# youmi-zym/GO-SLAM

Measured on NVIDIA H100. Metric: keyframe-BA-updates/s, higher is better.
Workload: dtype f16 corr (f32 accumulate) / f32 BA (f64 solve)

## Files before the change

go-slam_b200/csrc/ba.cu:

```cuda
#include "common.cuh"
#include <cstring>
#include "se3.cuh"
#include <algorithm>
#include <cstdio>
#include <mutex>
#include <cooperative_groups.h>

namespace {

constexpr int kTP = 128;
constexpr int kNRed = 27;
constexpr float kAlpha = 0.05f;

struct BaWs {
  int* slot_of_frame;
  int* kx;
  int* counts;
  int* row_ptr;
  int* edge_idx;
  int* entry_ptr;
  int* entry_code;
  int* pair_ptr;
  int* edge_j;
  float* Eij;
  float* Ei;
  float* Q;
  float* w;
  float* part;
  double* sys;
  double* chol;
  double* rhs;
  float* dx;
  int ntiles;
};

struct BaDims {
  int N, num, ht, wd, hw, t0, t1, P, n;
};

size_t ba_layout(const BaDims& d, void* base, size_t cap, BaWs* ws) {
  GsArena a(base, cap);
  const int ntiles = gs_cdiv(d.hw, kTP);
  BaWs w{};
  w.slot_of_frame = a.take<int>(d.num);
  w.kx = a.take<int>(d.num);
  w.counts = a.take<int>(8);
  w.row_ptr = a.take<int>(d.num + 1);
  w.edge_idx = a.take<int>(d.N > 0 ? d.N : 1);
  w.entry_ptr = a.take<int>(d.num + 1);
  w.entry_code = a.take<int>(d.num + d.N);
  w.pair_ptr = a.take<int>(d.num + 1);
  w.edge_j = a.take<int>(d.N > 0 ? d.N : 1);
  w.Eij = a.take<float>((size_t)(d.N > 0 ? d.N : 1) * 6 * d.hw);
  w.Ei = a.take<float>((size_t)d.num * 6 * d.hw);
  w.Q = a.take<float>((size_t)d.num * d.hw);
  w.w = a.take<float>((size_t)d.num * d.hw);
  w.part = a.take<float>((size_t)(d.N > 0 ? d.N : 1) * ntiles * (kTP / 32) * kNRed);
  w.sys = a.take<double>((size_t)d.n * d.n + d.n);
  w.chol = a.take<double>((size_t)d.n * d.n);
  w.rhs = a.take<double>(d.n > 0 ? d.n : 1);
  w.dx = a.take<float>((size_t)(d.P > 0 ? d.P : 1) * 6);
  w.ntiles = ntiles;
  if (ws) *ws = w;
  return a.off;
}

constexpr int kPrepThreads = 1024;
constexpr int kPrepMaxFrames = 4 * kPrepThreads;

__device__ int prep_excl_scan(int* a, int n, int* wsum ) {
  const int tid = threadIdx.x, lane = tid & 31, warp = tid >> 5;
  const int per = (n + (int)blockDim.x - 1) / (int)blockDim.x;
  const int base = tid * per;
  int loc[4], s = 0;
#pragma unroll
  for (int q = 0; q < 4; ++q) {
    loc[q] = s;
    if (q < per && base + q < n) s += a[base + q];
  }
  int inc = s;
#pragma unroll
  for (int o = 1; o < 32; o <<= 1) {
    const int t = __shfl_up_sync(0xffffffffu, inc, o);
    if (lane >= o) inc += t;
  }
  if (lane == 31) wsum[warp] = inc;
  __syncthreads();
  if (warp == 0) {
    const int w = lane < ((int)blockDim.x >> 5) ? wsum[lane] : 0;
    int winc = w;
#pragma unroll
    for (int o = 1; o < 32; o <<= 1) {
      const int t = __shfl_up_sync(0xffffffffu, winc, o);
      if (lane >= o) winc += t;
    }
    wsum[lane] = winc - w;
    if (lane == 31) wsum[32] = winc;
  }
  __syncthreads();
  const int off = wsum[warp] + inc - s;
#pragma unroll
  for (int q = 0; q < 4; ++q)
    if (q < per && base + q < n) a[base + q] = off + loc[q];
  const int total = wsum[32];
  __syncthreads();
  return total;
}

__global__ void __launch_bounds__(kPrepThreads)
ba_prep_kernel(const int64_t* __restrict__ ii, const int64_t* __restrict__ jj, BaDims d, BaWs ws, int zero,
               int eta_rows) {
  extern __shared__ int sm[];
  const int tid = threadIdx.x, nt = blockDim.x;
  if (zero) {
    const size_t nsys = (size_t)d.n * d.n + d.n;
    for (size_t i = tid; i < nsys; i += nt) ws.sys[i] = 0.0;
    if (tid == 0) ws.counts[3] = 0;
  }
  int* a = sm;
  int* b = sm + d.num;
  int* c = b + d.num + 1;
  int* wsum = c + d.num;
  for (int f = tid; f < d.num; f += nt) { a[f] = (f >= d.t0 && f < d.t1) ? 1 : 0; b[f] = 0; }
  __syncthreads();
  for (int e = tid; e < d.N; e += nt) {
    const int f = (int)ii[e];
    if (f >= 0 && f < d.num) { a[f] = 1; atomicAdd(&b[f], 1); }
    ws.edge_j[e] = (int)jj[e];
  }
  __syncthreads();
  for (int f = tid; f < d.num; f += nt) c[f] = a[f];
  __syncthreads();
  const int M = prep_excl_scan(c, d.num, wsum);
  for (int f = tid; f < d.num; f += nt) {
    if (a[f]) { ws.slot_of_frame[f] = c[f]; ws.kx[c[f]] = f; }
    else ws.slot_of_frame[f] = -1;
  }
  if (tid == 0) {
    ws.counts[0] = M;
    ws.counts[4] = (eta_rows == 0 || eta_rows == 1 || eta_rows == M || eta_rows == -d.num) ? 0 : 1;
  }
  const int n_listed = prep_excl_scan(b, d.num, wsum);
  if (tid == 0) b[d.num] = n_listed;
  __syncthreads();
  for (int f = tid; f <= d.num; f += nt) ws.row_ptr[f] = b[f];
  for (int e = tid; e < d.N; e += nt) {
    const int f = (int)ii[e];
    if (f < 0 || f >= d.num) continue;
    int rank = 0;
    for (int q = 0; q < e; ++q) rank += ((int)ii[q] == f);
    ws.edge_idx[b[f] + rank] = e;
  }
  __syncthreads();
  for (int k = tid; k < d.num; k += nt) {
    int ne = 0;
    if (k < M) {
      const int f = ws.kx[k];
      ne = (f >= d.t0 && f < d.t1) ? 1 : 0;
      for (int r = b[f]; r < b[f + 1]; ++r) {
        const int j = (int)jj[ws.edge_idx[r]];
        ne += (j >= d.t0 && j < d.t1) ? 1 : 0;
      }
    }
    a[k] = ne;
    c[k] = ne * (ne + 1) / 2;
  }
  __syncthreads();
  const int n_entries = prep_excl_scan(a, d.num, wsum);
  const int n_pairs = prep_excl_scan(c, d.num, wsum);
  for (int k = tid; k < M; k += nt) {
    const int f = ws.kx[k];
    int eo = a[k];
    ws.entry_ptr[k] = eo;
    ws.pair_ptr[k] = c[k];
    if (f >= d.t0 && f < d.t1) ws.entry_code[eo++] = -(f - d.t0 + 1);
    for (int r = b[f]; r < b[f + 1]; ++r) {
      const int e = ws.edge_idx[r];
      const int j = (int)jj[e];
      if (j >= d.t0 && j < d.t1) ws.entry_code[eo++] = e;
    }
  }
  if (tid == 0) {
    ws.entry_ptr[M] = n_entries;
    ws.pair_ptr[M] = n_pairs;
    ws.counts[1] = n_entries;
    ws.counts[2] = n_pairs;
  }
}

__device__ __forceinline__ float warp_transpose_reduce32(float (&v)[32], int lane) {
#pragma unroll
  for (int half = 16; half >= 1; half >>= 1) {
    const bool up = (lane & half) != 0;
#pragma unroll
    for (int i = 0; i < half; ++i) {
      const float send = up ? v[i] : v[i + half];
      const float keep = up ? v[i + half] : v[i];
      v[i] = keep + __shfl_xor_sync(0xffffffffu, send, half);
    }
  }
  return v[0];
}

struct BaIn {
  const float* poses; const float* disps; const float* intr; const float* disps_sens;
  const float* targets; const float* weights; const float* eta; int eta_rows;
  const int64_t* ii; const int64_t* jj;
};

__device__ __forceinline__ void linearize_tile(const BaIn& in, const BaDims& d, const BaWs& ws,
                                               int motion_only, int k, int wt) {
  const float* poses = in.poses; const float* disps = in.disps;
  const float* __restrict__ intr = in.intr; const float* __restrict__ disps_sens = in.disps_sens;
  const float* __restrict__ targets = in.targets; const float* __restrict__ weights = in.weights;
  const float* __restrict__ eta = in.eta; const int eta_rows = in.eta_rows;
  const int f = ws.kx[k];
  const int lane = threadIdx.x & 31;
  const int px = wt * 32 + lane;
  const bool act = px < d.hw;

  const float fx = intr[0], fy = intr[1], cx = intr[2], cy = intr[3];
  const float u = (float)(px % d.wd), v = (float)(px / d.wd);
  const float di = act ? disps[(size_t)f * d.hw + px] : 1.0f;
  float Xi[4] = {(u - cx) / fx, (v - cy) / fy, 1.0f, di};

  float C = 0.f, wz = 0.f;
  float Ei[6] = {0.f, 0.f, 0.f, 0.f, 0.f, 0.f};

  const int r0 = ws.row_ptr[f], r1 = ws.row_ptr[f + 1];
  float pi[7];
#pragma unroll
  for (int c = 0; c < 7; ++c) pi[c] = poses[7 * (size_t)f + c];
  int e1 = 0, j1 = f, e2 = 0, j2 = f;
  if (r0 < r1) { e1 = ws.edge_idx[r0]; j1 = ws.edge_j[e1]; }
  if (r0 + 1 < r1) { e2 = ws.edge_idx[r0 + 1]; j2 = ws.edge_j[e2]; }
  float nx[4] = {0.f, 0.f, 0.f, 0.f}, pn[7] = {0.f, 0.f, 0.f, 0.f, 0.f, 0.f, 1.f};
  if (r0 < r1) {
    if (act) {
      const size_t o = ((size_t)e1 * 2) * d.hw + px;
      nx[0] = targets[o]; nx[1] = targets[o + d.hw]; nx[2] = weights[o]; nx[3] = weights[o + d.hw];
    }
#pragma unroll
    for (int c = 0; c < 7; ++c) pn[c] = poses[7 * (size_t)j1 + c];
  }
  for (int r = r0; r < r1; ++r) {
    const int e = e1, jx = j1;
    const float tu = nx[0], tv = nx[1], qu = nx[2], qv = nx[3];
    float pj[7];
#pragma unroll
    for (int c = 0; c < 7; ++c) pj[c] = pn[c];
    e1 = e2; j1 = j2;
    if (r + 1 < r1) {
      if (act) {
        const size_t o = ((size_t)e1 * 2) * d.hw + px;
        nx[0] = targets[o]; nx[1] = targets[o + d.hw]; nx[2] = weights[o]; nx[3] = weights[o + d.hw];
      }
#pragma unroll
      for (int c = 0; c < 7; ++c) pn[c] = poses[7 * (size_t)j1 + c];
    }
    if (r + 2 < r1) { e2 = ws.edge_idx[r + 2]; j2 = ws.edge_j[e2]; }
    const bool stereo = (jx == f);
    GsSE3 G;
    if (stereo) {
      G.t[0] = -0.1f; G.t[1] = 0.f; G.t[2] = 0.f;
      G.q[0] = 0.f; G.q[1] = 0.f; G.q[2] = 0.f; G.q[3] = 1.f;
    } else {
      gs_rel(pi, pi + 3, pj, pj + 3, G);
    }

    float Xj[4];
    gs_act4(G, Xi, Xj);
    const float x = Xj[0], y = Xj[1], h = Xj[3];
    const bool behind = Xj[2] < GS_MIN_DEPTH;
    const float dd = behind ? 0.0f : __frcp_rn(Xj[2]);
    const float d2 = dd * dd;
    float wu = (behind || !act) ? 0.0f : (float)(.001 * (double)qu);
    float wv = (behind || !act) ? 0.0f : (float)(.001 * (double)qv);
    const float ru = tu - (fx * dd * x + cx);
    const float rv = tv - (fy * dd * y + cy);

    float Ju[6], Jv[6];
    Ju[0] = fx * (h * dd);       Ju[1] = fx * 0.f;
    Ju[2] = fx * (-x * h * d2);  Ju[3] = fx * (-x * y * d2);
    Ju[4] = fx * (1 + x * x * d2);  Ju[5] = fx * (-y * dd);
    Jv[0] = fy * 0.f;            Jv[1] = fy * (h * dd);
    Jv[2] = fy * (-y * h * d2);  Jv[3] = fy * (-1 - y * y * d2);
    Jv[4] = fy * (x * y * d2);   Jv[5] = fy * (x * dd);
    const float Jzu = fx * (G.t[0] * dd - G.t[2] * (x * d2));
    const float Jzv = fy * (G.t[1] * dd - G.t[2] * (y * d2));

    C += wu * Jzu * Jzu;  C += wv * Jzv * Jzv;
    wz += wu * ru * Jzu;  wz += wv * rv * Jzv;
    if (stereo) { wu = 0.f; wv = 0.f; }

    float val[32];
    {
      int l = 0;
#pragma unroll
      for (int a = 0; a < 6; ++a)
#pragma unroll
        for (int b = a; b < 6; ++b) val[l++] = wu * Ju[a] * Ju[b] + wv * Jv[a] * Jv[b];
#pragma unroll
      for (int a = 0; a < 6; ++a) val[21 + a] = wu * ru * Ju[a] + wv * rv * Jv[a];
#pragma unroll
      for (int a = kNRed; a < 32; ++a) val[a] = 0.f;
    }
    const float tot = warp_transpose_reduce32(val, lane);
    if (lane < kNRed)
      ws.part[((size_t)e * ws.ntiles * (kTP / 32) + wt) * kNRed + lane] = tot;

    if (!motion_only) {
      float Ee[6], Eii[6];
#pragma unroll
      for (int a = 0; a < 6; ++a) Ee[a] = wu * Jzu * Ju[a] + wv * Jzv * Jv[a];
      gs_adjT(G, Ee, Eii);
      if (act) {
#pragma unroll
        for (int a = 0; a < 6; ++a) {
          ws.Eij[((size_t)e * 6 + a) * d.hw + px] = Ee[a];
          Ei[a] -= Eii[a];
        }
      }
    }
  }

  if (!motion_only && act) {
    const float ds = disps_sens[(size_t)f * d.hw + px];
    const float m = (ds > 0.f) ? 1.0f : 0.0f;
    const int er = (eta_rows == 1) ? 0 : (eta_rows < 0 ? f : k);
    const float et = eta[(size_t)er * d.hw + px];
    C = C + m * kAlpha + (1.0f - m) * et;
    wz = wz - m * kAlpha * (di - ds);
    const size_t o = (size_t)k * d.hw + px;
    ws.Q[o] = 1.0f / C;
    ws.w[o] = wz;
#pragma unroll
    for (int a = 0; a < 6; ++a) ws.Ei[((size_t)k * 6 + a) * d.hw + px] = Ei[a];
  }
}

__global__ void __launch_bounds__(kTP)
ba_linearize_kernel(BaIn in, BaDims d, BaWs ws, int motion_only) {
  if ((int)blockIdx.y >= ws.counts[0] || ws.counts[4]) return;
  linearize_tile(in, d, ws, motion_only, blockIdx.y, blockIdx.x * (kTP / 32) + (threadIdx.x >> 5));
}

struct SysSmem {
  float red[8][64];
  double redd[8][32];
  double Hs[36], Ms[36], Ts[36], vs[6];
};

template <int NT>
__device__ __forceinline__ void system_items(const float* poses, const int64_t* __restrict__ ii,
                                             const int64_t* __restrict__ jj, const BaDims& d,
                                             const BaWs& ws, int motion_only, int bid, int nb,
                                             SysSmem& sm) {
  float (*red)[64] = sm.red;
  double* Hs = sm.Hs; double* Ms = sm.Ms; double* Ts = sm.Ts; double* vs = sm.vs;
  const int tid = threadIdx.x, lane = tid & 31, warp = tid >> 5;
  const int M = ws.counts[0];
  const int npairs = motion_only ? 0 : ws.counts[2];
  constexpr int kChunk = 4 * NT;
  const int nchunk = (d.hw + kChunk - 1) / kChunk;
  double* H = ws.sys;
  double* bvec = ws.sys + (size_t)d.n * d.n;

  for (int e = nb - 1 - bid; e < d.N; e += nb) {
    const int ix = (int)ii[e], jx = (int)jj[e];
    const int pi = ix - d.t0, pj = jx - d.t0;
    const bool vi_ok = pi >= 0 && pi < d.P, vj_ok = pj >= 0 && pj < d.P;
    if ((!vi_ok && !vj_ok) || ix < 0 || ix >= d.num) continue;
    {
      double ps = 0.0;
      if (lane < kNRed) {
        const int nparts = ws.ntiles * (kTP / 32);
        const float* pp = ws.part + (size_t)e * nparts * kNRed + lane;
#pragma unroll 8
        for (int t = warp; t < nparts; t += NT / 32) ps += (double)pp[(size_t)t * kNRed];
      }
      sm.redd[warp][lane] = ps;
    }
    __syncthreads();
    if (tid < kNRed) {
      double s = 0.0;
#pragma unroll
      for (int wq = 0; wq < NT / 32; ++wq) s += sm.redd[wq][tid];
      if (tid < 21) {
        int a = 0, l = tid;
        while (l >= 6 - a) { l -= 6 - a; ++a; }
        const int b = a + l;
        Hs[a * 6 + b] = s; Hs[b * 6 + a] = s;
      } else {
        vs[tid - 21] = s;
      }
    }
    if (tid >= 32 && tid < 38) {
      const int c = tid - 32;
      GsSE3 G;
      gs_edge_pose(poses, ix, jx, G);
      float X[6] = {0.f, 0.f, 0.f, 0.f, 0.f, 0.f}, Y[6];
      X[c] = 1.0f;
      gs_adjT(G, X, Y);
      for (int r = 0; r < 6; ++r) Ms[r * 6 + c] = (double)Y[r];
    }
    __syncthreads();
    if (tid < 36) {
      const int r = tid / 6, c = tid % 6;
      double s = 0.0;
      for (int q = 0; q < 6; ++q) s += Ms[r * 6 + q] * Hs[q * 6 + c];
      Ts[tid] = s;
    }
    __syncthreads();
    if (tid < 36) {
      const int r = tid / 6, c = tid % 6;
      if (vi_ok) {
        double s = 0.0;
        for (int q = 0; q < 6; ++q) s += Ts[r * 6 + q] * Ms[c * 6 + q];
        atomicAdd(&H[(size_t)(6 * pi + r) * d.n + 6 * pi + c], s);
      }
      if (vi_ok && vj_ok) {
        atomicAdd(&H[(size_t)(6 * pi + r) * d.n + 6 * pj + c], -Ts[r * 6 + c]);
        atomicAdd(&H[(size_t)(6 * pj + r) * d.n + 6 * pi + c], -Ts[c * 6 + r]);
      }
      if (vj_ok) atomicAdd(&H[(size_t)(6 * pj + r) * d.n + 6 * pj + c], Hs[r * 6 + c]);
    } else if (tid >= 64 && tid < 70) {
      const int r = tid - 64;
      if (vj_ok) atomicAdd(&bvec[6 * pj + r], vs[r]);
      if (vi_ok) {
        double s = 0.0;
        for (int q = 0; q < 6; ++q) s += Ms[r * 6 + q] * vs[q];
        atomicAdd(&bvec[6 * pi + r], -s);
      }
    }
    __syncthreads();
  }

  const int total = npairs * nchunk;
  const int per = (total + nb - 1) / nb;
  const int u0 = bid * per;
  const int u1 = min(total, u0 + per);
  int cur = -1, pa = 0, pb = 0;
  bool diag = false;
  const float* Ea = nullptr; const float* Eb = nullptr; const float* Qk = nullptr; const float* wk = nullptr;
  float acc[64];
  auto flush = [&]() {
    float lo32[32], hi32[32];
#pragma unroll
    for (int i = 0; i < 32; ++i) { lo32[i] = acc[i]; hi32[i] = acc[32 + i]; }
    const float s0 = warp_transpose_reduce32(lo32, lane);
    const float s1 = warp_transpose_reduce32(hi32, lane);
    red[warp][lane] = s0;
    red[warp][32 + lane] = s1;
    __syncthreads();
    if (tid < 42) {
      double s = 0.0;
#pragma unroll
      for (int wq = 0; wq < NT / 32; ++wq) s += (double)red[wq][tid];
      if (tid < 36) {
        const int r = tid / 6, c = tid % 6;
        atomicAdd(&H[(size_t)(6 * pa + r) * d.n + 6 * pb + c], -s);
        if (!diag) atomicAdd(&H[(size_t)(6 * pb + c) * d.n + 6 * pa + r], -s);
      } else {
        atomicAdd(&bvec[6 * pa + (tid - 36)], -s);
      }
    }
    __syncthreads();
  };
  for (int u = u0; u < u1; ++u) {
    const int p = u / nchunk;
    const int px0 = (u - p * nchunk) * kChunk;
    const int px1 = min(d.hw, px0 + kChunk);
    if (p != cur) {
      if (cur >= 0) flush();
      cur = p;
      int k;
      if (M <= 32) {
        const int v = lane < M ? ws.pair_ptr[lane] : 0x7fffffff;
        k = __popc(__ballot_sync(0xffffffffu, v <= p)) - 1;
      } else {
        int lo = 0, hi = M;
        while (hi - lo > 1) {
          const int mid = (lo + hi) >> 1;
          if (ws.pair_ptr[mid] <= p) lo = mid; else hi = mid;
        }
        k = lo;
      }
      const int e0 = ws.entry_ptr[k];
      const int ne = ws.entry_ptr[k + 1] - e0;
      int q = p - ws.pair_ptr[k];
      int a = 0;
      while (q >= ne - a) { q -= ne - a; ++a; }
      const int b = a + q;
      const int ca = ws.entry_code[e0 + a];
      const int cb = ws.entry_code[e0 + b];
      Ea = (ca >= 0) ? ws.Eij + (size_t)ca * 6 * d.hw : ws.Ei + (size_t)k * 6 * d.hw;
      Eb = (cb >= 0) ? ws.Eij + (size_t)cb * 6 * d.hw : ws.Ei + (size_t)k * 6 * d.hw;
      pa = (ca >= 0) ? ws.edge_j[ca] - d.t0 : -ca - 1;
      pb = (cb >= 0) ? ws.edge_j[cb] - d.t0 : -cb - 1;
      Qk = ws.Q + (size_t)k * d.hw;
      wk = ws.w + (size_t)k * d.hw;
      diag = a == b;
#pragma unroll
      for (int i = 0; i < 64; ++i) acc[i] = 0.f;
    }
    float qv[kChunk / NT], wv[kChunk / NT], ea[kChunk / NT][6], eb[kChunk / NT][6];
#pragma unroll
    for (int v = 0; v < kChunk / NT; ++v) {
      const int px = px0 + tid + v * NT;
      const bool ok = px < px1;
      qv[v] = ok ? Qk[px] : 0.f;
      wv[v] = (ok && diag) ? wk[px] : 0.f;
#pragma unroll
      for (int r = 0; r < 6; ++r) {
        ea[v][r] = ok ? Ea[(size_t)r * d.hw + px] : 0.f;
        eb[v][r] = ok ? Eb[(size_t)r * d.hw + px] : 0.f;
      }
    }
#pragma unroll
    for (int v = 0; v < kChunk / NT; ++v) {
#pragma unroll
      for (int r = 0; r < 6; ++r) ea[v][r] *= qv[v];
#pragma unroll
      for (int r = 0; r < 6; ++r)
#pragma unroll
        for (int c = 0; c < 6; ++c) acc[r * 6 + c] += ea[v][r] * eb[v][c];
#pragma unroll
      for (int r = 0; r < 6; ++r) acc[36 + r] += ea[v][r] * wv[v];
    }
  }
  if (cur >= 0) flush();
}

__global__ void __launch_bounds__(256)
ba_system_kernel(const float* poses, const int64_t* __restrict__ ii,
                 const int64_t* __restrict__ jj, BaDims d, BaWs ws, int motion_only) {
  __shared__ SysSmem sm;
  if (ws.counts[4]) return;
  system_items<256>(poses, ii, jj, d, ws, motion_only, blockIdx.x, gridDim.x, sm);
}

constexpr int kMaxPeers = 8;
struct SysSrc {
  const double* p[kMaxPeers];
  int n;
  const unsigned* flags;
  unsigned epoch;
  int* timeout;
};
struct PeerRows {
  float* p[kMaxPeers];
  int n;
};

__device__ __forceinline__ double sys_at(const SysSrc& s, size_t i) {
  double x[kMaxPeers];
#pragma unroll
  for (int r = 0; r < kMaxPeers; ++r) x[r] = r < s.n ? __ldcg(s.p[r] + i) : 0.0;
  double v = x[0];
#pragma unroll
  for (int r = 1; r < kMaxPeers; ++r) v += x[r];
  return v;
}

__device__ __forceinline__ void peer_wait(const unsigned* flags, int n, unsigned epoch, int* timeout) {
  if (n > 1 && (int)threadIdx.x < n) {
    const long long t0 = clock64();
    unsigned v;
    do {
      asm volatile("ld.acquire.sys.global.u32 %0, [%1];" : "=r"(v) : "l"(flags + threadIdx.x) : "memory");
      if ((int)(v - epoch) >= 0) break;
      if (clock64() - t0 > (1ll << 32)) { if (timeout) *timeout = 1; break; }
    } while (true);
  }
  __syncthreads();
}

__global__ void ba_peer_wait_kernel(const unsigned* flags, int n, unsigned epoch, int* timeout) {
  peer_wait(flags, n, epoch, timeout);
}

__global__ void ba_peer_signal_kernel(PeerRows flag_rows, int slot, unsigned epoch) {
  __threadfence_system();
  if ((int)threadIdx.x < flag_rows.n) {
    unsigned* dst = reinterpret_cast<unsigned*>(flag_rows.p[threadIdx.x]) + slot;
    asm volatile("st.release.sys.global.u32 [%0], %1;" ::"l"(dst), "r"(epoch) : "memory");
  }
}

__device__ __forceinline__ void solve_finish(float* poses, const BaDims& d, const BaWs& ws,
                                             const double* x, int fail, float* dx_out,
                                             int* status_out, int tid, int nt) {
  for (int i = tid; i < d.n; i += nt) {
    const float val = fail ? 0.0f : (float)x[i];
    ws.dx[i] = val;
    if (dx_out) dx_out[i] = val;
  }
  if (tid == 0 && status_out) *status_out = fail;
}

__device__ __forceinline__ void bad_argument_step(const BaDims& d, const BaWs& ws, float* dx_out,
                                                  int* status_out, int tid, int nt) {
  for (int i = tid; i < d.n; i += nt) {
    ws.dx[i] = 0.f;
    if (dx_out) dx_out[i] = 0.f;
  }
  if (tid == 0 && status_out) *status_out = 2;
}

__device__ __forceinline__ void retract_poses(float* poses, const BaDims& d, const BaWs& ws, int tid,
                                              int nt) {
  for (int k = tid; k < d.P; k += nt) {
    float* p = poses + 7 * (size_t)(d.t0 + k);
    float t1[3], q1[4];
    gs_retr(ws.dx + 6 * k, p, p + 3, t1, q1);
    p[0] = t1[0]; p[1] = t1[1]; p[2] = t1[2];
    p[3] = q1[0]; p[4] = q1[1]; p[5] = q1[2]; p[6] = q1[3];
  }
}

struct SolveSmem {
  double Lblk[16][15];
  double xs[6];
  int failed;
};

#ifdef GOSLAM_BA_PROBE
__device__ long long g_solve_probe[8];
__device__ int g_phase_cycles[2][1024];
#define SOLVE_PROBE(slot) do { if (threadIdx.x == 0) g_solve_probe[slot] = clock64(); } while (0)
#else
#define SOLVE_PROBE(slot) do {} while (0)
#endif

__device__ __forceinline__ void solve_small(float* poses, const BaDims& d, const BaWs& ws,
                                            const SysSrc& sys_in, float lm, float ep, float* dx_out,
                                            int* status_out, double* smd, SolveSmem& ss) {
  double* xs = ss.xs;
  int& failed = ss.failed;
  const int n = d.n, P = d.P, tid = threadIdx.x, lane = tid & 31;
  double* __restrict__ A = smd;
  double* __restrict__ invd = smd + (size_t)(n + 1) * n;
  SOLVE_PROBE(0);
  float pose_old[7] = {0.f, 0.f, 0.f, 0.f, 0.f, 0.f, 1.f};
  if (tid < P) {
#pragma unroll
    for (int c = 0; c < 7; ++c) pose_old[c] = poses[7 * (size_t)(d.t0 + tid) + c];
  }
  {
    const int tot = (n + 1) * n;
    for (int base = 0; base < tot; base += 128 * 16) {
      double v[16];
#pragma unroll
      for (int u = 0; u < 16; ++u) {
        const int idx = base + tid + 128 * u;
        const int r = idx / n, c = idx - r * n;
        v[u] = (idx < tot && (c <= r || r == n)) ? sys_at(sys_in, idx) : 0.0;
      }
#pragma unroll
      for (int u = 0; u < 16; ++u) {
        const int idx = base + tid + 128 * u;
        const int r = idx / n, c = idx - r * n;
        if (idx < tot && (c <= r || r == n)) {
          double val = v[u];
          if (r == c) val += (double)ep + (double)lm * val;
          A[idx] = val;
        }
      }
    }
  }
  if (tid == 0) failed = 0;
  __syncthreads();
  SOLVE_PROBE(1);

  bool bad = false;
  for (int jb = 0; jb < P; ++jb) {
    const int j0 = 6 * jb;
    double l[6][6];
#pragma unroll
    for (int r = 0; r < 6; ++r)
#pragma unroll
      for (int c = 0; c <= r; ++c) l[r][c] = A[(j0 + r) * n + j0 + c];
#pragma unroll
    for (int k = 0; k < 6; ++k) {
      double dkk = l[k][k];
#pragma unroll
      for (int m = 0; m < k; ++m) dkk -= l[k][m] * l[k][m];
      bad = bad || !(dkk > 0.0);
      const double inv = rsqrt(dkk);
      l[k][k] = inv;
#pragma unroll
      for (int r = k + 1; r < 6; ++r) {
// ... 385 lines not shown
          double* out = rowp + c * 36 + a * 6;
#pragma unroll
          for (int b = 0; b < 6; ++b) {
            double v = out[b];
#pragma unroll
            for (int k = 0; k < 6; ++k) v -= li[k] * Lc[b * 6 + k];
            acc[b] = v;
          }
#pragma unroll
          for (int b = 0; b < 6; ++b) out[b] = acc[b];
        }
      }
      for (int it = ut; it < (P - 1 - jb) * 6; it += un) {
        const int c = jb + 1 + it / 6, b = it % 6;
        const double* Lc = panel + (size_t)c * 36 + b * 6;
        double v = rhs[6 * c + b];
#pragma unroll
        for (int k = 0; k < 6; ++k) v -= xs[k] * Lc[k];
        rhs[6 * c + b] = v;
      }
    }
    CL_PROBE(2);
    cluster.sync();
    CL_PROBE(3);
  }

  {
    for (int jb = P - 1; jb >= 0; --jb) {
      const int owner = jb % kCl, lo = jb / kCl;
      if (q == owner) {
        const double* Ld = rows + cl_row_off(q, lo) + jb * 36;
        if (tid == 0) {
          double v6[6], x[6];
#pragma unroll
          for (int k = 0; k < 6; ++k) {
            const double s01 = inbox[0 * 6 + k] + inbox[1 * 6 + k], s23 = inbox[2 * 6 + k] + inbox[3 * 6 + k];
            const double s45 = inbox[4 * 6 + k] + inbox[5 * 6 + k], s67 = inbox[6 * 6 + k] + inbox[7 * 6 + k];
            v6[k] = rhs[6 * jb + k] - ((s01 + s23) + (s45 + s67));
          }
          int nf = 0;
#pragma unroll
          for (int k = 0; k < 6; ++k) {
            double v = Ld[k * 6 + k] * v6[k];
#pragma unroll
            for (int m = k + 1; m < 6; ++m) v += Ld[m * 6 + k] * v6[m];
            x[k] = v;
            nf |= !isfinite(v);
          }
#pragma unroll
          for (int k = 0; k < 6; ++k) { xs[k] = x[k]; ws.dx[6 * jb + k] = (float)x[k]; }
          if (nf) failed = 1;
        }
        __syncthreads();
        const double* rowp = rows + cl_row_off(q, lo);
        const int cpush = jb < kCl ? jb : kCl;
        if (tid < cpush * 6) {
          const int c = jb - 1 - tid / 6, k = tid % 6;
          const double* blk = rowp + c * 36;
          double v = ps[6 * c + k];
#pragma unroll
          for (int m = 0; m < 6; ++m) v += blk[m * 6 + k] * xs[m];
          ps[6 * c + k] = v;
          cluster.map_shared_rank(inbox, c % kCl)[q * 6 + k] = v;
        }
        for (int it = tid; it < (jb - cpush) * 6; it += kClT) {
          const int c = it / 6, k = it % 6;
          const double* blk = rowp + c * 36;
          double v = ps[6 * c + k];
#pragma unroll
          for (int m = 0; m < 6; ++m) v += blk[m * 6 + k] * xs[m];
          ps[6 * c + k] = v;
        }
      }
      CL_PROBE(5);
      cluster.sync();
      CL_PROBE(6);
    }
  }
#ifdef GOSLAM_BA_PROBE
  if (tid == 0 && (q == 0 || q == 5))
    printf("[cluster solve probe cta %d, P=%d] panel+push %lld | barrier1 %lld | update (factor hidden) %lld | barrier2 %lld | "
           "backward work %lld | backward barrier %lld (cycles)\n", q, P, pc[0], pc[1], pc[2], pc[3], pc[5], pc[6]);
#endif
  if (q == 0) {
    __shared__ int any_fail;
    if (tid == 0) {
      int f = 0;
      for (int oq = 0; oq < kCl; ++oq) f |= *cluster.map_shared_rank(&failed, oq);
      any_fail = f;
    }
    __syncthreads();
    const int fail = any_fail;
    for (int i = tid; i < n; i += kClT) {
      const float val = fail ? 0.0f : ws.dx[i];
      ws.dx[i] = val;
      if (dx_out) dx_out[i] = val;
    }
    if (tid == 0 && status_out) *status_out = fail;
    __syncthreads();
    retract_poses(poses, d, ws, tid, kClT);
  }
  cluster.sync();
}

__device__ __forceinline__ void backsub_tile(float* disps, const BaDims& d, const BaWs& ws,
                                             int owner_lo, int owner_hi, float* dz_out, int k,
                                             int wt, const PeerRows* peers = nullptr) {
  const int f = ws.kx[k];
  if (f < owner_lo || f >= owner_hi) return;
  const int px = wt * 32 + (threadIdx.x & 31);
  if (px >= d.hw) return;
  float acc = 0.f;
  {
    const int ix = f - d.t0;
    if (ix > 0 && ix < d.P) {
      float dw = 0.f;
#pragma unroll
      for (int a = 0; a < 6; ++a) dw += ws.Ei[((size_t)k * 6 + a) * d.hw + px] * ws.dx[6 * ix + a];
      acc += dw;
    }
  }
  for (int r = ws.row_ptr[f]; r < ws.row_ptr[f + 1]; ++r) {
    const int e = ws.edge_idx[r];
    const int ix = ws.edge_j[e] - d.t0;
    if (ix <= 0 || ix >= d.P) continue;
    float dw = 0.f;
#pragma unroll
    for (int a = 0; a < 6; ++a) dw += ws.Eij[((size_t)e * 6 + a) * d.hw + px] * ws.dx[6 * ix + a];
    acc += dw;
  }
  const size_t o = (size_t)k * d.hw + px;
  const float dz = ws.Q[o] * (ws.w[o] - acc);
  const float nv = disps[(size_t)f * d.hw + px] + dz;
  disps[(size_t)f * d.hw + px] = nv;
  if (peers)
    for (int r = 0; r < peers->n; ++r)
      if (peers->p[r] != disps) peers->p[r][(size_t)f * d.hw + px] = nv;
  if (dz_out) dz_out[(size_t)f * d.hw + px] = dz;
}

__global__ void __launch_bounds__(kTP)
ba_backsub_kernel(float* disps, BaDims d, BaWs ws, int owner_lo, int owner_hi, float* dz_out, const PeerRows peers) {
  if ((int)blockIdx.y >= ws.counts[0] || ws.counts[4]) return;
  backsub_tile(disps, d, ws, owner_lo, owner_hi, dz_out, blockIdx.y, blockIdx.x * (kTP / 32) + (threadIdx.x >> 5),
               peers.n > 1 ? &peers : nullptr);
}

#ifdef GOSLAM_BA_PROBE
#define BA_PROBE(slot) do { if (threadIdx.x == 0 && blockIdx.x == 0) probe[slot] = clock64(); } while (0)
#else
#define BA_PROBE(slot) do {} while (0)
#endif

__device__ __forceinline__ void grid_barrier(unsigned* counter, unsigned& epoch) {
  __syncthreads();
  ++epoch;
  if (threadIdx.x == 0) {
    __threadfence();
    atomicAdd(counter, 1u);
    const unsigned target = epoch * gridDim.x;
    unsigned v;
    do {
      asm volatile("ld.acquire.gpu.global.u32 %0, [%1];" : "=r"(v) : "l"(counter) : "memory");
    } while (v < target);
    __threadfence();
  }
  __syncthreads();
}

__global__ void __launch_bounds__(kTP)
ba_persistent_kernel(float* poses, float* disps, BaIn in, BaDims d, BaWs ws, int iterations, float lm,
                     float ep, int motion_only, float* dx_out, float* dz_out, int* status_out,
                     unsigned* barrier) {
  extern __shared__ double smd[];
  __shared__ SysSmem sys_sm;
  __shared__ SolveSmem solve_sm;
  unsigned epoch = 0;
#ifdef GOSLAM_BA_PROBE
  __shared__ long long probe[8];
#endif
  const int M = ws.counts[0];
  const int nwt = ws.ntiles * (kTP / 32);
  const int units = M * nwt;
  const int ufirst = (threadIdx.x >> 5) * gridDim.x + blockIdx.x, ustep = (kTP / 32) * gridDim.x;
  const size_t nsys = (size_t)d.n * d.n + d.n;
  if (dz_out) {
    const size_t ndz = (size_t)d.num * d.hw;
    for (size_t i = (size_t)blockIdx.x * kTP + threadIdx.x; i < ndz; i += (size_t)gridDim.x * kTP) dz_out[i] = 0.f;
  }
  if (ws.counts[4]) {
    if (blockIdx.x == 0) {
      bad_argument_step(d, ws, dx_out, nullptr, threadIdx.x, kTP);
      if (status_out) for (int it = threadIdx.x; it < iterations; it += kTP) status_out[it] = 2;
    }
    return;
  }
  for (int it = 0; it < iterations; ++it) {
    BA_PROBE(0);
#ifdef GOSLAM_BA_PROBE
    const long long tl0 = clock64();
#endif
    for (int u = ufirst; u < units; u += ustep) {
      const int k = u / nwt, wt = u - k * nwt;
      if (it > 0 && !motion_only) backsub_tile(disps, d, ws, 0, d.num, dz_out, k, wt);
      linearize_tile(in, d, ws, motion_only, k, wt);
    }
#ifdef GOSLAM_BA_PROBE
    if (threadIdx.x == 0 && blockIdx.x < 1024) g_phase_cycles[0][blockIdx.x] = (int)(clock64() - tl0);
#endif
    BA_PROBE(1);
    grid_barrier(barrier, epoch);
    BA_PROBE(2);
#ifdef GOSLAM_BA_PROBE
    const long long ts0 = clock64();
#endif
    system_items<kTP>(poses, in.ii, in.jj, d, ws, motion_only, blockIdx.x, gridDim.x, sys_sm);
#ifdef GOSLAM_BA_PROBE
    if (threadIdx.x == 0 && blockIdx.x < 1024) g_phase_cycles[1][blockIdx.x] = (int)(clock64() - ts0);
#endif
    BA_PROBE(3);
    grid_barrier(barrier, epoch);
    BA_PROBE(4);
    if (blockIdx.x == 0) {
      SysSrc local{};
      local.p[0] = ws.sys; local.n = 1;
      solve_small(poses, d, ws, local, lm, ep, dx_out, status_out ? status_out + it : nullptr, smd,
                  solve_sm);
      __syncthreads();
      for (size_t i = threadIdx.x; i < nsys; i += kTP) ws.sys[i] = 0.0;
    }
    BA_PROBE(5);
    grid_barrier(barrier, epoch);
    BA_PROBE(6);
#ifdef GOSLAM_BA_PROBE
    if (threadIdx.x == 0 && blockIdx.x == 0 && it == iterations - 1) {
      for (int ph = 0; ph < 2; ++ph) {
        int mx = 0, arg = 0;
        for (int b = 0; b < (int)gridDim.x && b < 1024; ++b)
          if (g_phase_cycles[ph][b] > mx) { mx = g_phase_cycles[ph][b]; arg = b; }
        printf("[phase %d] slowest block %d: %d cycles; blocks 0/100/200/244/250/270/290/295: %d %d %d %d %d %d %d %d\n", ph, arg,
               mx, g_phase_cycles[ph][0], g_phase_cycles[ph][100], g_phase_cycles[ph][200], g_phase_cycles[ph][244],
               g_phase_cycles[ph][250], g_phase_cycles[ph][270], g_phase_cycles[ph][290], g_phase_cycles[ph][295]);
      }
    }
    if (threadIdx.x == 0 && blockIdx.x == 0)
      printf("[solve probe it=%d] load %lld | factor %lld | backward %lld | finish+retract %lld\n", it,
             g_solve_probe[1] - g_solve_probe[0], g_solve_probe[2] - g_solve_probe[1],
             g_solve_probe[3] - g_solve_probe[2], g_solve_probe[4] - g_solve_probe[3]);
    if (threadIdx.x == 0 && blockIdx.x == 0)
      printf("[ba probe it=%d] linearize %lld | barrier %lld | system %lld | barrier %lld | solve %lld | barrier %lld (cycles)\n",
             it, probe[1] - probe[0], probe[2] - probe[1], probe[3] - probe[2], probe[4] - probe[3],
             probe[5] - probe[4], probe[6] - probe[5]);
#endif
  }
  if (!motion_only)
    for (int u = ufirst; u < units; u += ustep) {
      const int k = u / nwt, wt = u - k * nwt;
      backsub_tile(disps, d, ws, 0, d.num, dz_out, k, wt);
    }
}

bool make_dims(int N, int num, int ht, int wd, int t0, int t1, BaDims* d) {
  if (N < 0 || num <= 0 || num > 4096 || ht <= 0 || wd <= 0) return false;
  d->N = N; d->num = num; d->ht = ht; d->wd = wd; d->hw = ht * wd;
  d->t0 = t0; d->t1 = t1; d->P = t1 - t0 > 0 ? t1 - t0 : 0; d->n = 6 * d->P;
  if (t0 < 0 || t1 > num) return false;
  return true;
}

constexpr int kSmemSolveMaxN = 160;
constexpr int kWarpSolveMaxN = 96;
constexpr int kMaxDevices = 64;
constexpr size_t kClusterSmemMax = 226 * 1024;

struct BaDevice {
  bool ready = false;
  int sms = 0;
  int blocks_per_sm = 0;
};

void ba_persistent_kernel_attrs(BaDevice* dv, int dev) {
  int occ = 0, coop = 0;
  const size_t smem_max = ((size_t)kWarpSolveMaxN * kWarpSolveMaxN + 2 * kWarpSolveMaxN) * sizeof(double);
  cudaDeviceGetAttribute(&dv->sms, cudaDevAttrMultiProcessorCount, dev);
  cudaDeviceGetAttribute(&coop, cudaDevAttrCooperativeLaunch, dev);
  cudaFuncSetAttribute(ba_persistent_kernel, cudaFuncAttributeMaxDynamicSharedMemorySize, (int)smem_max);
  cudaOccupancyMaxActiveBlocksPerMultiprocessor(&occ, ba_persistent_kernel, kTP, smem_max);
  constexpr int kWant = 2;
  dv->blocks_per_sm = (!coop || occ < 1) ? 0 : (occ > kWant ? kWant : occ);
}

inline size_t prep_smem_bytes(int num) { return ((size_t)3 * num + 1 + 33) * sizeof(int); }

const BaDevice& ba_device() {
  static BaDevice table[kMaxDevices];
  static std::mutex mu;
  int dev = 0;
  cudaGetDevice(&dev);
  if (dev < 0 || dev >= kMaxDevices) dev = 0;
  std::lock_guard<std::mutex> lock(mu);
  BaDevice& dv = table[dev];
  if (!dv.ready) {
    cudaFuncSetAttribute(ba_prep_kernel, cudaFuncAttributeMaxDynamicSharedMemorySize, (int)prep_smem_bytes(kPrepMaxFrames));
    cudaFuncSetAttribute(ba_solve_kernel, cudaFuncAttributeMaxDynamicSharedMemorySize,
                         (int)(((size_t)kSmemSolveMaxN * kSmemSolveMaxN + kSmemSolveMaxN) * 8));
    cudaFuncSetAttribute(ba_solve_warp_kernel, cudaFuncAttributeMaxDynamicSharedMemorySize,
                         (int)(((size_t)kWarpSolveMaxN * kWarpSolveMaxN + 2 * kWarpSolveMaxN) * 8));
    cudaFuncSetAttribute(ba_solve_cluster_kernel, cudaFuncAttributeMaxDynamicSharedMemorySize,
                         (int)kClusterSmemMax);
    ba_persistent_kernel_attrs(&dv, dev);
    dv.ready = true;
  }
  return dv;
}


int launch_phase1(const float* poses, const float* disps, const float* intr,
                  const float* disps_sens, const float* targets, const float* weights,
                  const float* eta, int eta_rows, const int64_t* ii, const int64_t* jj,
                  const BaDims& d, const BaWs& ws, int motion_only, bool prep, cudaStream_t st) {
  const BaIn in{poses, disps, intr, disps_sens, targets, weights, eta, eta_rows, ii, jj};
  if (prep) {
    ba_prep_kernel<<<1, kPrepThreads, prep_smem_bytes(d.num), st>>>(ii, jj, d, ws, 0, motion_only ? 0 : eta_rows);
    GS_CHECK_LAUNCH();
  }
  cudaMemsetAsync(ws.sys, 0, ((size_t)d.n * d.n + d.n) * sizeof(double), st);
  if (d.N > 0) {
    dim3 grid(ws.ntiles, d.num);
    ba_linearize_kernel<<<grid, kTP, 0, st>>>(in, d, ws, motion_only);
    GS_CHECK_LAUNCH();
  } else if (!motion_only) {
    dim3 grid(ws.ntiles, d.num);
    ba_linearize_kernel<<<grid, kTP, 0, st>>>(in, d, ws, motion_only);
    GS_CHECK_LAUNCH();
  }
  ba_system_kernel<<<kNumSms * 4, 256, 0, st>>>(poses, ii, jj, d, ws, motion_only);
  GS_CHECK_LAUNCH();
  return GOSLAM_OK;
}

int launch_phase2(float* poses, float* disps, const SysSrc& sys_in,
                  const BaDims& d, const BaWs& ws, float lm, float ep, int motion_only,
                  int owner_lo, int owner_hi, float* dx_out, float* dz_out, int* status_out,
                  cudaStream_t st, const PeerRows& peer_rows = PeerRows{}) {
  const BaDevice& dv = ba_device();
  (void)dv;
  if (d.n <= kWarpSolveMaxN) {
    const size_t smem = ((size_t)d.n * d.n + 2 * d.n) * sizeof(double);
    ba_solve_warp_kernel<<<1, 128, smem, st>>>(poses, d, ws, sys_in, lm, ep, dx_out, status_out);
  } else if (cl_smem_bytes(d.P) <= kClusterSmemMax) {
    cudaLaunchConfig_t cfg = {};
    cfg.gridDim = dim3(kCl);
    cfg.blockDim = dim3(kClT);
    cfg.dynamicSmemBytes = cl_smem_bytes(d.P);
    cfg.stream = st;
    cudaLaunchAttribute attr[1];
    attr[0].id = cudaLaunchAttributeClusterDimension;
    attr[0].val.clusterDim.x = kCl; attr[0].val.clusterDim.y = 1; attr[0].val.clusterDim.z = 1;
    cfg.attrs = attr;
    cfg.numAttrs = 1;
    const int rows_doubles = (int)cl_rows_doubles(d.P);
    const cudaError_t le = cudaLaunchKernelEx(&cfg, ba_solve_cluster_kernel, poses, d, ws, sys_in, lm, ep,
                                              rows_doubles, dx_out, status_out);
    if (le != cudaSuccess) { gs_note_cuda_error(le); return GOSLAM_ELAUNCH; }
  } else {
    const int use_smem = d.n <= kSmemSolveMaxN;
    const size_t smem = use_smem ? ((size_t)d.n * d.n + d.n) * sizeof(double) : 0;
    const int threads = d.n <= kSmemSolveMaxN ? 256 : 1024;
    ba_solve_kernel<<<1, threads, smem, st>>>(poses, d, ws, sys_in, lm, ep, use_smem, dx_out,
                                              status_out);
  }
  GS_CHECK_LAUNCH();
  if (!motion_only) {
    dim3 grid(ws.ntiles, d.num);
    ba_backsub_kernel<<<grid, kTP, 0, st>>>(disps, d, ws, owner_lo, owner_hi, dz_out, peer_rows);
    GS_CHECK_LAUNCH();
  }
  return GOSLAM_OK;
}

}

extern "C" {

size_t goslam_ba_workspace_bytes(int N, int num, int ht, int wd, int t0, int t1) {
  BaDims d;
  if (!make_dims(N, num, ht, wd, t0, t1, &d)) return 0;
  return ba_layout(d, nullptr, 0, nullptr) + 256;
}

size_t goslam_ba_system_doubles(int t0, int t1) {
  const size_t n = 6 * (size_t)(t1 > t0 ? t1 - t0 : 0);
  return n * n + n;
}

int goslam_ba(float* poses, float* disps, const float* intrinsics, const float* disps_sens,
              const float* targets, const float* weights, const float* eta, int eta_rows,
              const int64_t* ii, const int64_t* jj, int N, int num, int ht, int wd, int t0,
              int t1, int iterations, float lm, float ep, int motion_only, float* dx_out,
              float* dz_out, int* status_out, void* workspace, size_t workspace_bytes,
              void* stream) {
  BaDims d;
  if (!make_dims(N, num, ht, wd, t0, t1, &d)) return GOSLAM_EINVAL;
  if (!motion_only && (eta == nullptr || eta_rows == 0)) return GOSLAM_EINVAL;
  if (d.P == 0 || iterations <= 0) return GOSLAM_OK;
  BaWs ws;
  const size_t need = ba_layout(d, workspace, workspace_bytes, &ws);
  if (workspace == nullptr || need > workspace_bytes) return GOSLAM_EWORKSPACE;
  cudaStream_t st = (cudaStream_t)stream;
#ifdef GOSLAM_BA_FORCE_MULTIKERNEL
  constexpr bool multi_kernel = true;
#else
  constexpr bool multi_kernel = false;
#endif
  if (d.n <= kWarpSolveMaxN && !multi_kernel) {
    const BaDevice& dv = ba_device();
    const int blocks_per_sm = dv.blocks_per_sm, sms = dv.sms;
    const size_t smem = ((size_t)d.n * d.n + 2 * d.n) * sizeof(double);
    if (blocks_per_sm > 0) {
      ba_prep_kernel<<<1, kPrepThreads, prep_smem_bytes(d.num), st>>>(ii, jj, d, ws, 1, motion_only ? 0 : eta_rows);
      GS_CHECK_LAUNCH();
      unsigned* barrier = reinterpret_cast<unsigned*>(ws.counts + 3);
      BaIn in{poses, disps, intrinsics, disps_sens, targets, weights, eta, eta_rows, ii, jj};
      BaDims dd = d;
      BaWs wsv = ws;
      void* args[] = {&poses, &disps, &in, &dd, &wsv, &iterations, &lm, &ep, &motion_only,
                      &dx_out, &dz_out, &status_out, &barrier};
      const cudaError_t le = cudaLaunchCooperativeKernel((const void*)ba_persistent_kernel,
                                                         dim3(sms * blocks_per_sm), dim3(kTP), args, smem, st);
      if (le != cudaSuccess) { gs_note_cuda_error(le); return GOSLAM_ELAUNCH; }
      return GOSLAM_OK;
    }
  }
  if (dz_out) cudaMemsetAsync(dz_out, 0, (size_t)num * d.hw * sizeof(float), st);
  for (int it = 0; it < iterations; ++it) {
    int rc = launch_phase1(poses, disps, intrinsics, disps_sens, targets, weights, eta, eta_rows,
                           ii, jj, d, ws, motion_only, it == 0, st);
    if (rc) return rc;
    SysSrc local{};
    local.p[0] = ws.sys; local.n = 1;
    rc = launch_phase2(poses, disps, local, d, ws, lm, ep, motion_only, 0, num, dx_out,
                       dz_out, status_out ? status_out + it : nullptr, st);
    if (rc) return rc;
  }
  return GOSLAM_OK;
}

int goslam_ba_phase1(const float* poses, const float* disps, const float* intrinsics,
                     const float* disps_sens, const float* targets, const float* weights,
                     const float* eta, int eta_rows, const int64_t* ii, const int64_t* jj, int N,
                     int num, int ht, int wd, int t0, int t1, int motion_only, double* system,
                     void* workspace, size_t workspace_bytes, void* stream) {
  BaDims d;
  if (!make_dims(N, num, ht, wd, t0, t1, &d)) return GOSLAM_EINVAL;
  if (d.P == 0) return GOSLAM_OK;
  BaWs ws;
  const size_t need = ba_layout(d, workspace, workspace_bytes, &ws);
  if (workspace == nullptr || need > workspace_bytes) return GOSLAM_EWORKSPACE;
  cudaStream_t st = (cudaStream_t)stream;
  int rc = launch_phase1(poses, disps, intrinsics, disps_sens, targets, weights, eta, eta_rows, ii,
                         jj, d, ws, motion_only, true, st);
  if (rc) return rc;
  if (system != ws.sys)
    cudaMemcpyAsync(system, ws.sys, ((size_t)d.n * d.n + d.n) * sizeof(double),
                    cudaMemcpyDeviceToDevice, st);
  return GOSLAM_OK;
}

int goslam_ba_phase2(float* poses, float* disps, const double* system, int N, int num, int ht,
                     int wd, int t0, int t1, float lm, float ep, int motion_only, int owner_lo,
                     int owner_hi, float* dx_out, float* dz_out, int* status_out, void* workspace,
                     size_t workspace_bytes, void* stream) {
  BaDims d;
  if (!make_dims(N, num, ht, wd, t0, t1, &d)) return GOSLAM_EINVAL;
  if (d.P == 0) return GOSLAM_OK;
  BaWs ws;
  const size_t need = ba_layout(d, workspace, workspace_bytes, &ws);
  if (workspace == nullptr || need > workspace_bytes) return GOSLAM_EWORKSPACE;
  SysSrc local{};
  local.p[0] = system; local.n = 1;
  return launch_phase2(poses, disps, local, d, ws, lm, ep, motion_only, owner_lo, owner_hi, dx_out,
                       dz_out, status_out, (cudaStream_t)stream);
}

static bool peers_ok(const goslam_ba_peers* p) {
  if (!p || p->world < 1 || p->world > kMaxPeers || p->rank < 0 || p->rank >= p->world || p->epoch == 0) return false;
  for (int r = 0; r < p->world; ++r)
    if (!p->system[r] || !p->flags[r] || !p->disps[r]) return false;
  return true;
}

int goslam_ba_phase1_peers(const float* poses, const float* intrinsics, const float* disps_sens, const float* targets,
                           const float* weights, const float* eta, int eta_rows, const int64_t* ii, const int64_t* jj,
                           int N, int num, int ht, int wd, int t0, int t1, int motion_only,
                           const goslam_ba_peers* peers, void* workspace, size_t workspace_bytes, void* stream) {
  BaDims d;
  if (!make_dims(N, num, ht, wd, t0, t1, &d) || !peers_ok(peers)) return GOSLAM_EINVAL;
  if (d.P == 0) return GOSLAM_OK;
  BaWs ws;
  const size_t need = ba_layout(d, workspace, workspace_bytes, &ws);
  if (workspace == nullptr || need > workspace_bytes) return GOSLAM_EWORKSPACE;
  cudaStream_t st = (cudaStream_t)stream;
  const int W = peers->world, me = peers->rank;
  if (W > 1) {
    ba_peer_wait_kernel<<<1, 32, 0, st>>>(peers->flags[me] + W, W, peers->epoch - 1, peers->timeout);
    GS_CHECK_LAUNCH();
  }
  int rc = launch_phase1(poses, peers->disps[me], intrinsics, disps_sens, targets, weights, eta, eta_rows, ii, jj, d, ws,
                         motion_only, true, st);
  if (rc) return rc;
  if (peers->system[me] != ws.sys)
    cudaMemcpyAsync(peers->system[me], ws.sys, ((size_t)d.n * d.n + d.n) * sizeof(double), cudaMemcpyDeviceToDevice, st);
  if (W > 1) {
    PeerRows rows{};
    rows.n = W;
    for (int r = 0; r < W; ++r) rows.p[r] = reinterpret_cast<float*>(peers->flags[r]);
    ba_peer_signal_kernel<<<1, 32, 0, st>>>(rows, me, peers->epoch);
    GS_CHECK_LAUNCH();
  }
  return GOSLAM_OK;
}

int goslam_ba_phase2_peers(float* poses, int N, int num, int ht, int wd, int t0, int t1, float lm, float ep,
                           int motion_only, int owner_lo, int owner_hi, const goslam_ba_peers* peers, float* dx_out,
                           float* dz_out, int* status_out, void* workspace, size_t workspace_bytes, void* stream) {
  BaDims d;
  if (!make_dims(N, num, ht, wd, t0, t1, &d) || !peers_ok(peers)) return GOSLAM_EINVAL;
  if (d.P == 0) return GOSLAM_OK;
  BaWs ws;
  const size_t need = ba_layout(d, workspace, workspace_bytes, &ws);
  if (workspace == nullptr || need > workspace_bytes) return GOSLAM_EWORKSPACE;
  cudaStream_t st = (cudaStream_t)stream;
  const int W = peers->world, me = peers->rank;
  SysSrc src{};
  src.n = W;
  for (int r = 0; r < W; ++r) src.p[r] = peers->system[r];
  src.flags = peers->flags[me]; src.epoch = peers->epoch; src.timeout = peers->timeout;
  PeerRows rows{};
  rows.n = W;
  for (int r = 0; r < W; ++r) rows.p[r] = peers->disps[r];
  const int rc = launch_phase2(poses, peers->disps[me], src, d, ws, lm, ep, motion_only, owner_lo, owner_hi, dx_out, dz_out,
                               status_out, st, rows);
  if (rc) return rc;
  if (W > 1) {
    PeerRows frows{};
    frows.n = W;
    for (int r = 0; r < W; ++r) frows.p[r] = reinterpret_cast<float*>(peers->flags[r]);
    ba_peer_signal_kernel<<<1, 32, 0, st>>>(frows, W + me, peers->epoch);
    GS_CHECK_LAUNCH();
  }
  return GOSLAM_OK;
}

int goslam_ba_peers_wait(const goslam_ba_peers* peers, void* stream) {
  if (!peers_ok(peers)) return GOSLAM_EINVAL;
  if (peers->world > 1) {
    ba_peer_wait_kernel<<<1, 32, 0, (cudaStream_t)stream>>>(peers->flags[peers->rank] + peers->world, peers->world,
                                                            peers->epoch, peers->timeout);
    GS_CHECK_LAUNCH();
  }
  return GOSLAM_OK;
}

int goslam_peer_alloc(size_t bytes, void** ptr, void* handle_out) {
  if (!ptr || !handle_out || bytes == 0) return GOSLAM_EINVAL;
  void* q = nullptr;
  cudaError_t e = cudaMalloc(&q, bytes);
  if (e == cudaSuccess) e = cudaMemset(q, 0, bytes);
  cudaIpcMemHandle_t h;
  if (e == cudaSuccess) e = cudaIpcGetMemHandle(&h, q);
  if (e != cudaSuccess) { gs_note_cuda_error(e); if (q) cudaFree(q); return GOSLAM_ELAUNCH; }
  memcpy(handle_out, &h, sizeof(h));
  *ptr = q;
  return GOSLAM_OK;
}

int goslam_peer_free(void* ptr) {
  if (!ptr) return GOSLAM_EINVAL;
  const cudaError_t e = cudaFree(ptr);
  if (e != cudaSuccess) { gs_note_cuda_error(e); return GOSLAM_ELAUNCH; }
// ... 21 lines not shown
```

Measured before the change: 1502.

## Double-buffer BA system and replace post-system grid barriers with arrive/publish flags

The persistent BA kernel now alternates between two Hessian/rhs buffers, so each iteration's next buffer is zeroed in parallel during linearization instead of by block 0 after the solve. The two full grid barriers around the solve become a counter that only block 0 waits on and a release-published 'solved' flag that the other blocks poll. This removes one grid-wide round trip and the serial zeroing pass from the critical path, at the cost of an extra system-sized workspace buffer and more intricate memory-ordering logic. Smaller edits add a templated unroll of the transpose reduction and a compile-time knob for blocks per SM.

Result: faster. 1582, median of 6 (+5.4%).

```diff
diff --git a/go-slam_b200/csrc/ba.cu b/go-slam_b200/csrc/ba.cu
--- a/go-slam_b200/csrc/ba.cu
+++ b/go-slam_b200/csrc/ba.cu
@@ -28,6 +28,7 @@
   float* w;
   float* part;
   double* sys;
+  double* sys_alt;
   double* chol;
   double* rhs;
   float* dx;
@@ -57,6 +58,7 @@
   w.w = a.take<float>((size_t)d.num * d.hw);
   w.part = a.take<float>((size_t)(d.N > 0 ? d.N : 1) * ntiles * (kTP / 32) * kNRed);
   w.sys = a.take<double>((size_t)d.n * d.n + d.n);
+  w.sys_alt = a.take<double>((size_t)d.n * d.n + d.n);
   w.chol = a.take<double>((size_t)d.n * d.n);
   w.rhs = a.take<double>(d.n > 0 ? d.n : 1);
   w.dx = a.take<float>((size_t)(d.P > 0 ? d.P : 1) * 6);
@@ -115,7 +117,7 @@
   if (zero) {
     const size_t nsys = (size_t)d.n * d.n + d.n;
     for (size_t i = tid; i < nsys; i += nt) ws.sys[i] = 0.0;
-    if (tid == 0) ws.counts[3] = 0;
+    if (tid == 0) { ws.counts[3] = 0; ws.counts[5] = 0; ws.counts[6] = 0; }
   }
   int* a = sm;
   int* b = sm + d.num;
@@ -188,17 +190,20 @@
   }
 }
 
+template <int HALF>
+__device__ __forceinline__ void transpose_reduce_step(float (&v)[32], int lane) {
+  const bool up = (lane & HALF) != 0;
+#pragma unroll
+  for (int i = 0; i < HALF; ++i) {
+    const float send = up ? v[i] : v[i + HALF];
+    const float keep = up ? v[i + HALF] : v[i];
+    v[i] = keep + __shfl_xor_sync(0xffffffffu, send, HALF);
+  }
+  if constexpr (HALF > 1) transpose_reduce_step<HALF / 2>(v, lane);
+}
+
 __device__ __forceinline__ float warp_transpose_reduce32(float (&v)[32], int lane) {
-#pragma unroll
-  for (int half = 16; half >= 1; half >>= 1) {
-    const bool up = (lane & half) != 0;
-#pragma unroll
-    for (int i = 0; i < half; ++i) {
-      const float send = up ? v[i] : v[i + half];
-      const float keep = up ? v[i + half] : v[i];
-      v[i] = keep + __shfl_xor_sync(0xffffffffu, send, half);
-    }
-  }
+  transpose_reduce_step<16>(v, lane);
   return v[0];
 }
 
@@ -354,8 +359,8 @@
 template <int NT>
 __device__ __forceinline__ void system_items(const float* poses, const int64_t* __restrict__ ii,
                                              const int64_t* __restrict__ jj, const BaDims& d,
-                                             const BaWs& ws, int motion_only, int bid, int nb,
-                                             SysSmem& sm) {
+                                             const BaWs& ws, double* sys, int motion_only, int bid,
+                                             int nb, SysSmem& sm) {
   float (*red)[64] = sm.red;
   double* Hs = sm.Hs; double* Ms = sm.Ms; double* Ts = sm.Ts; double* vs = sm.vs;
   const int tid = threadIdx.x, lane = tid & 31, warp = tid >> 5;
@@ -363,8 +368,8 @@
   const int npairs = motion_only ? 0 : ws.counts[2];
   constexpr int kChunk = 4 * NT;
   const int nchunk = (d.hw + kChunk - 1) / kChunk;
-  double* H = ws.sys;
-  double* bvec = ws.sys + (size_t)d.n * d.n;
+  double* H = sys;
+  double* bvec = sys + (size_t)d.n * d.n;
 
   for (int e = nb - 1 - bid; e < d.N; e += nb) {
     const int ix = (int)ii[e], jx = (int)jj[e];
@@ -399,9 +404,11 @@
       const int c = tid - 32;
       GsSE3 G;
       gs_edge_pose(poses, ix, jx, G);
-      float X[6] = {0.f, 0.f, 0.f, 0.f, 0.f, 0.f}, Y[6];
-      X[c] = 1.0f;
+      float X[6], Y[6];
+#pragma unroll
+      for (int r = 0; r < 6; ++r) X[r] = (r == c) ? 1.0f : 0.0f;
       gs_adjT(G, X, Y);
+#pragma unroll
       for (int r = 0; r < 6; ++r) Ms[r * 6 + c] = (double)Y[r];
     }
     __syncthreads();
@@ -537,7 +544,7 @@
                  const int64_t* __restrict__ jj, BaDims d, BaWs ws, int motion_only) {
   __shared__ SysSmem sm;
   if (ws.counts[4]) return;
-  system_items<256>(poses, ii, jj, d, ws, motion_only, blockIdx.x, gridDim.x, sm);
+  system_items<256>(poses, ii, jj, d, ws, ws.sys, motion_only, blockIdx.x, gridDim.x, sm);
 }
 
 constexpr int kMaxPeers = 8;
@@ -1229,26 +1236,43 @@
 #define BA_PROBE(slot) do {} while (0)
 #endif
 
-__device__ __forceinline__ void grid_barrier(unsigned* counter, unsigned& epoch) {
+__device__ __forceinline__ void block_arrive(unsigned* counter) {
   __syncthreads();
-  ++epoch;
   if (threadIdx.x == 0) {
     __threadfence();
     atomicAdd(counter, 1u);
-    const unsigned target = epoch * gridDim.x;
+  }
+}
+
+__device__ __forceinline__ void block_wait_at_least(const unsigned* word, unsigned target) {
+  if (threadIdx.x == 0) {
     unsigned v;
     do {
-      asm volatile("ld.acquire.gpu.global.u32 %0, [%1];" : "=r"(v) : "l"(counter) : "memory");
+      asm volatile("ld.acquire.gpu.global.u32 %0, [%1];" : "=r"(v) : "l"(word) : "memory");
     } while (v < target);
     __threadfence();
   }
   __syncthreads();
+}
+
+__device__ __forceinline__ void block_publish(unsigned* word, unsigned value) {
+  __syncthreads();
+  if (threadIdx.x == 0) {
+    __threadfence();
+    asm volatile("st.release.gpu.global.u32 [%0], %1;" ::"l"(word), "r"(value) : "memory");
+  }
+}
+
+__device__ __forceinline__ void grid_barrier(unsigned* counter, unsigned& epoch) {
+  block_arrive(counter);
+  ++epoch;
+  block_wait_at_least(counter, epoch * gridDim.x);
 }
 
 __global__ void __launch_bounds__(kTP)
 ba_persistent_kernel(float* poses, float* disps, BaIn in, BaDims d, BaWs ws, int iterations, float lm,
                      float ep, int motion_only, float* dx_out, float* dz_out, int* status_out,
-                     unsigned* barrier) {
+                     unsigned* barrier, unsigned* arrived, unsigned* solved) {
   extern __shared__ double smd[];
   __shared__ SysSmem sys_sm;
   __shared__ SolveSmem solve_sm;
@@ -1277,10 +1301,15 @@
 #ifdef GOSLAM_BA_PROBE
     const long long tl0 = clock64();
 #endif
+    double* const sys = (it & 1) ? ws.sys_alt : ws.sys;
     for (int u = ufirst; u < units; u += ustep) {
       const int k = u / nwt, wt = u - k * nwt;
       if (it > 0 && !motion_only) backsub_tile(disps, d, ws, 0, d.num, dz_out, k, wt);
       linearize_tile(in, d, ws, motion_only, k, wt);
+    }
+    if (it + 1 < iterations) {
+      double* const next = (it & 1) ? ws.sys : ws.sys_alt;
+      for (size_t i = (size_t)blockIdx.x * kTP + threadIdx.x; i < nsys; i += (size_t)gridDim.x * kTP) next[i] = 0.0;
     }
 #ifdef GOSLAM_BA_PROBE
     if (threadIdx.x == 0 && blockIdx.x < 1024) g_phase_cycles[0][blockIdx.x] = (int)(clock64() - tl0);
@@ -1291,23 +1320,24 @@
 #ifdef GOSLAM_BA_PROBE
     const long long ts0 = clock64();
 #endif
-    system_items<kTP>(poses, in.ii, in.jj, d, ws, motion_only, blockIdx.x, gridDim.x, sys_sm);
+    system_items<kTP>(poses, in.ii, in.jj, d, ws, sys, motion_only, blockIdx.x, gridDim.x, sys_sm);
 #ifdef GOSLAM_BA_PROBE
     if (threadIdx.x == 0 && blockIdx.x < 1024) g_phase_cycles[1][blockIdx.x] = (int)(clock64() - ts0);
 #endif
     BA_PROBE(3);
-    grid_barrier(barrier, epoch);
-    BA_PROBE(4);
+    block_arrive(arrived);
     if (blockIdx.x == 0) {
+      block_wait_at_least(arrived, (unsigned)(it + 1) * gridDim.x);
+      BA_PROBE(4);
       SysSrc local{};
-      local.p[0] = ws.sys; local.n = 1;
+      local.p[0] = sys; local.n = 1;
       solve_small(poses, d, ws, local, lm, ep, dx_out, status_out ? status_out + it : nullptr, smd,
                   solve_sm);
-      __syncthreads();
-      for (size_t i = threadIdx.x; i < nsys; i += kTP) ws.sys[i] = 0.0;
-    }
-    BA_PROBE(5);
-    grid_barrier(barrier, epoch);
+      BA_PROBE(5);
+      block_publish(solved, it + 1);
+    } else {
+      block_wait_at_least(solved, it + 1);
+    }
     BA_PROBE(6);
 #ifdef GOSLAM_BA_PROBE
     if (threadIdx.x == 0 && blockIdx.x == 0 && it == iterations - 1) {
@@ -1325,7 +1355,7 @@
              g_solve_probe[1] - g_solve_probe[0], g_solve_probe[2] - g_solve_probe[1],
              g_solve_probe[3] - g_solve_probe[2], g_solve_probe[4] - g_solve_probe[3]);
     if (threadIdx.x == 0 && blockIdx.x == 0)
-      printf("[ba probe it=%d] linearize %lld | barrier %lld | system %lld | barrier %lld | solve %lld | barrier %lld (cycles)\n",
+      printf("[ba probe it=%d] linearize %lld | barrier %lld | system %lld | wait for arrivals %lld | solve %lld | publish %lld (cycles)\n",
              it, probe[1] - probe[0], probe[2] - probe[1], probe[3] - probe[2], probe[4] - probe[3],
              probe[5] - probe[4], probe[6] - probe[5]);
 #endif
@@ -1363,7 +1393,10 @@
   cudaDeviceGetAttribute(&coop, cudaDevAttrCooperativeLaunch, dev);
   cudaFuncSetAttribute(ba_persistent_kernel, cudaFuncAttributeMaxDynamicSharedMemorySize, (int)smem_max);
   cudaOccupancyMaxActiveBlocksPerMultiprocessor(&occ, ba_persistent_kernel, kTP, smem_max);
-  constexpr int kWant = 2;
+#ifndef GOSLAM_BA_BLOCKS_PER_SM
+#define GOSLAM_BA_BLOCKS_PER_SM 2
+#endif
+  constexpr int kWant = GOSLAM_BA_BLOCKS_PER_SM;
   dv->blocks_per_sm = (!coop || occ < 1) ? 0 : (occ > kWant ? kWant : occ);
 }
 
@@ -1498,11 +1531,13 @@
       ba_prep_kernel<<<1, kPrepThreads, prep_smem_bytes(d.num), st>>>(ii, jj, d, ws, 1, motion_only ? 0 : eta_rows);
       GS_CHECK_LAUNCH();
       unsigned* barrier = reinterpret_cast<unsigned*>(ws.counts + 3);
+      unsigned* arrived = reinterpret_cast<unsigned*>(ws.counts + 5);
+      unsigned* solved = reinterpret_cast<unsigned*>(ws.counts + 6);
       BaIn in{poses, disps, intrinsics, disps_sens, targets, weights, eta, eta_rows, ii, jj};
       BaDims dd = d;
       BaWs wsv = ws;
       void* args[] = {&poses, &disps, &in, &dd, &wsv, &iterations, &lm, &ep, &motion_only,
-                      &dx_out, &dz_out, &status_out, &barrier};
+                      &dx_out, &dz_out, &status_out, &barrier, &arrived, &solved};
       const cudaError_t le = cudaLaunchCooperativeKernel((const void*)ba_persistent_kernel,
                                                          dim3(sms * blocks_per_sm), dim3(kTP), args, smem, st);
       if (le != cudaSuccess) { gs_note_cuda_error(le); return GOSLAM_ELAUNCH; }
```
